# VITA-Group/CV_A-FAN

Measured on AMD Instinct MI355X. Metric: images/sec (whole node) A-FAN K=5 train step, ResNet-18/CIFAR-10, higher is better.
Workload: dtype bf16; 1 GPU; resnet18 CIFAR-10-shape A-FAN K=5 bf16, batch 256/GPU, perturb_idx 6, internal layout nhwc, 1xMI355X per rank (BASELINE configs[1]); global_batch=256, parallelism=dp1, hipgraph=True, in_launch_batchnorm=True

## Files before the change

### cv_a-fan_amd/_lib.py

```python
import ctypes as C
import os

_HERE = os.path.dirname(os.path.abspath(__file__))
LIB_PATH = os.environ.get("AFAN_HIP_LIB") or os.path.join(_HERE, "libafan_hip.so")

AFAN_F32, AFAN_BF16 = 0, 1
AFAN_NCHW, AFAN_NHWC = 0, 1
_ERRORS = {-1: "AFAN_EDTYPE (unknown dtype code)", -2: "AFAN_EALIGN (misaligned pointer)",
           -3: "AFAN_ESHAPE (bad sizes)", -4: "AFAN_ENULL (required pointer is NULL)",
           -5: "AFAN_ELAYOUT (unknown layout code)"}

_p, _i, _l, _f = C.c_void_p, C.c_int, C.c_int64, C.c_float

SIGNATURES = {
    "afan_version": (_i, []),
    "afan_arch": (C.c_char_p, []),
    "afan_pgd_step": (_i, [_p, _p, _i, _p, _p, _l, _f, _f, _i, _p]),
    "afan_tensor_clamp": (_i, [_p, _p, _p, _l, _p]),
    "afan_norms_workspace_floats": (_l, [_l, _l]),
    "afan_pgd_step_norms": (_i, [_p, _p, _i, _p, _p, _l, _l, _f, _f, _i, _p, _p, _p, _p]),
    "afan_perturb_norms": (_i, [_p, _p, _l, _l, _p, _p, _p, _p]),
    "afan_axpy_noise": (_i, [_p, _p, _l, _f, _p, _p]),
    "afan_mix_feature": (_i, [_p, _p, _p, _l, _l, _l, _f, _i, _p]),
    "afan_mix_feature_nhwc": (_i, [_p, _p, _p, _l, _l, _l, _f, _i, _p]),
# ... 113 lines not shown
    "afan_roi_align_bwd_ws": (_i, [_p, _p, _p, _i, _i, _l, _l, _l, _l, _l, _i, _i, _f, _i, _p, _p]),
    "afan_transpose_weights": (_i, [_p, _p, _p, _i, _l, _p]),
    "afan_sgd_step": (_i, [_p, _p, _p, _p, _l, _p, _f, _f, _f, _i, _p]),
    "afan_sgd_step_guarded": (_i, [_p, _p, _p, _p, _l, _p, _f, _f, _f, _i, _p, _p]),
    "afan_guarded_copy": (_i, [_p, _p, _l, _p, _p, _p]),
    "afan_occupy_cus": (_i, [_i, _i, _i, _p]),
    "afan_cast_bf16": (_i, [_p, _p, _l, _p]),
    "afan_pgd_init": (_i, [_p, _i, _p, _p, _p, _l, _p]),
    "afan_normalize_nchw": (_i, [_p, _p, _i, _i, _l, _l, _l, _p, _p, _p]),
    "afan_profile_enable": (_i, [_i]),
    "afan_profile_collect": (_i, [C.c_char_p, C.POINTER(_l), C.POINTER(C.c_double), C.POINTER(C.c_double),
                                  C.POINTER(C.c_double), _i]),
    "afan_profile_event_overhead": (_i, [_i, C.POINTER(_f), _p]),
    "afan_conv_trace": (_i, [_i]),
    "afan_conv_trace_read": (_i, [C.POINTER(_l), C.c_char_p, _i]),
}

_lib = None


class AfanLibraryError(RuntimeError):
    pass


def load():
    global _lib
    if _lib is not None:
        return _lib
    if not os.path.exists(LIB_PATH):
        raise AfanLibraryError(
# ... 18 lines not shown
```

### cv_a-fan_amd/csrc/afan_conv.hip

```cpp
#include "afan_common.h"
#include "afan_conv_c64.h"
#include "afan_conv_stem.h"
#include "afan_conv_params.h"
#include <stdlib.h>

#ifndef AFAN_CONV_DRES_EARLY
#define AFAN_CONV_DRES_EARLY 1
#endif
#ifndef AFAN_CONV_FRAG_BATCH
#define AFAN_CONV_FRAG_BATCH 4
#endif

using namespace afan;
using namespace afan_conv;

namespace afan_nhwc {
int acc_slot_count(int64_t C);
int64_t acc_doubles(int64_t C);
int set_running_updates(int n);
}

namespace {

typedef __bf16 bf16x8 __attribute__((ext_vector_type(8)));
// ... 58 lines not shown

template <int KG, int BR> struct HaloSched {
    static constexpr int s(int t) { return (t < 0 || t >= 7) ? 0 : KG / 7 + (t < KG % 7 ? 1 : 0); }
    static constexpr int g0(int t) { int g = 0; for (int i = 0; i < t; ++i) g += s(i); return g; }
    static constexpr int slot(int tp, bool more) { return tp < 0 ? BR : ((tp + 3 < 9 || more) ? BR : 0) + (more ? s(tp) : 0); }
    static constexpr int wait(int t, bool more) { return slot(t - 1, more) + slot(t - 2, more); }
};

template <int KG, int BR> struct HaloSched5 {
    static constexpr int s(int t) { return (t < 0 || t >= 5) ? 0 : KG / 5 + (t < KG % 5 ? 1 : 0); }
    static constexpr int g0(int t) { int g = 0; for (int i = 0; i < t; ++i) g += s(i); return g; }
    static constexpr int slot(int tp, bool more) { return tp < 0 ? BR : ((tp + 5 < 9 || more) ? BR : 0) + (more ? s(tp) : 0); }
    static constexpr int wait(int t, bool more) { return slot(t - 1, more) + slot(t - 2, more) + slot(t - 3, more); }
};

template <int BM, int BN, int PF, int WM, int WN, int PW = 0, int FBT = AFAN_CONV_FRAG_BATCH, int HL = 0, bool GS = false, bool BF = false>
__device__ __forceinline__ void conv_igemm_body(const ConvP& pp) {
    static_assert(!(BF && GS), "in-launch BatchNorm: one image group");
    AFAN_PHASE(0);
    constexpr int NW = WM * WN;
    constexpr int THREADS = 64 * (NW + PW);
    constexpr int STG = PW ? 64 * PW : THREADS;
    constexpr int RPP = STG / 8;
    const ConvClass& cc = pp.cls[blockIdx.z];
    const uint32_t Wg = (uint32_t)cc.Wg, Hg = (uint32_t)cc.Hg;
    const uint32_t M = (uint32_t)pp.N * Hg * Wg;
    const uint32_t m0 = blockIdx.y * BM;
    if (m0 >= M) {
        if (pp.stats && threadIdx.x < BN && (int)(blockIdx.x * BN + threadIdx.x) < pp.Co) {
            const int64_t G = (int64_t)gridDim.y * gridDim.z, slot = (int64_t)blockIdx.z * gridDim.y + blockIdx.y;
            const int c = blockIdx.x * BN + threadIdx.x;
            pp.stats[((int64_t)0 * pp.Co + c) * G + slot] = 0.f;
            pp.stats[((int64_t)1 * pp.Co + c) * G + slot] = 0.f;
// ... 14 lines not shown

    const int tid = threadIdx.x, lane = tid & 63;
    const int wave = PW ? __builtin_amdgcn_readfirstlane(tid >> 6) : tid >> 6;
    const int wr = wave / WN, wc = wave % WN;
    const bool producer = PW && wave >= NW;
    const int stid = PW ? tid - 64 * NW : tid, swave = PW ? wave - NW : wave;
    const int n0 = blockIdx.x * BN;
    const int T = cc.T, Ci = pp.Ci, Hi = pp.Hi, Wi = pp.Wi;
    int tdh[MAX_TAPS], tdw[MAX_TAPS];
#pragma unroll
    for (int t = 0; t < MAX_TAPS; ++t) {
        tdh[t] = HL ? 0 : cc.dh[t];
        tdw[t] = HL ? 0 : cc.dw[t];
    }
    const int tap0_w = cc.wofs[0], tap0_a = cc.aofs[0], tap0_h = cc.dh[0], tap0_d = cc.dw[0];

    const __amdgpu_buffer_rsrc_t xr = __builtin_amdgcn_make_buffer_rsrc(
        const_cast<uint16_t*>(pp.x), 0, (int)((int64_t)pp.N * Hi * Wi * Ci * 2 + pp.a_extra), 0x00020000);
    const int w_row_stride = pp.multi ? pp.w_rs[blockIdx.z] : pp.w_row_stride;
    const __amdgpu_buffer_rsrc_t wrs = __builtin_amdgcn_make_buffer_rsrc(
        const_cast<uint16_t*>(pp.w + pp.w_off[blockIdx.z]), 0, (int)((int64_t)pp.Co * w_row_stride * 2), 0x00020000);
    constexpr uint32_t OOB = 0x80000000u;

    const int piece = GLDS ? ((stid & 7) ^ ((stid >> 4) & 7)) : (stid & 7);
    const int row0 = stid >> 3;
    uint32_t a_off[A_ROWS];
    uint32_t a_valid[A_ROWS];
#pragma unroll
    for (int i = 0; i < A_ROWS; ++i) {
        const uint32_t m = m0 + row0 + RPP * i;
        a_off[i] = 0;
        a_valid[i] = 0;
        if (!HL && m < M && (!PW || producer)) {
            const uint32_t t1 = m / Wg, wg = m - t1 * Wg;
            const uint32_t n = t1 / Hg, hg = t1 - n * Hg;
            const int hi0 = (int)hg * pp.in_s, wi0 = (int)wg * pp.in_s;
            a_off[i] = (((n * Hi + hi0) * Wi + wi0) * Ci + piece * 8) * 2u;
            uint32_t v = 0;
#pragma unroll
            for (int t = 0; t < MAX_TAPS; ++t)
                if ((t < T) & ((uint32_t)(hi0 + tdh[t]) < (uint32_t)Hi) & ((uint32_t)(wi0 + tdw[t]) < (uint32_t)Wi)) v |= 1u << t;
            a_valid[i] = v;
        }
    }
    __shared__ float coef_s[3][BN];
    float cv0 = 0.f, cv1 = 0.f, cv2 = 0.f;
    if (tid < BN) {
        const int c = n0 + tid < pp.Co ? n0 + tid : 0;
        const uint32_t half_ = (uint32_t)(pp.N / 2) * Hg * Wg;
        const int64_t o_ = c + (m0 >= half_ ? pp.coef_gofs : 0);
        const int64_t o0_ = o_ + ((pp.coef_mask & 8) ? pp.shift_off[blockIdx.z] : 0);
        cv0 = pp.coef[0][o0_];
        cv1 = pp.coef[1][o_];
        cv2 = pp.coef[2][o_];
    }
    auto late_prologue = [&]() {
        for (int r = tid; r < BM; r += THREADS) {
            const uint32_t m = m0 + r;
            int off = -1;
            if (m < M) {
                const uint32_t t1 = m / Wg, wg = m - t1 * Wg;
                const uint32_t n = t1 / Hg, hg = t1 - n * Hg;
                off = (int)(((n * pp.Ho + hg * pp.out_s + cc.out_h0) * pp.Wo + wg * pp.out_s + cc.out_w0) * pp.Co);
            }
            out_off[r] = off;
        }
        if (tid < BN) {
            const int mask_ = pp.coef_mask;
            coef_s[0][tid] = (mask_ & 1) ? cv0 : 0.f;
            coef_s[1][tid] = (mask_ & 2) ? cv1 : 0.f;
            coef_s[2][tid] = (mask_ & 4) ? cv2 : 0.f;
        }
    };
    const uint32_t b_off = ((uint32_t)(n0 + row0) * w_row_stride + piece * 8) * 2u;
    const int b_rows_ok = pp.Co - n0 - row0;
    const uint32_t b_row32 = (uint32_t)RPP * w_row_stride * 2u;

    f32x16 acc[NI][MI];
#pragma unroll
    for (int j = 0; j < NI; ++j)
#pragma unroll
        for (int i = 0; i < MI; ++i)
#pragma unroll
            for (int r = 0; r < 16; ++r) acc[j][i][r] = 0.f;

    const int chunks = (Ci + BK - 1) / BK;
    const int KS = T * chunks;
    const bool last_ok = (chunks - 1) * BK + piece * 8 < Ci;
    u32x4 ra0[A_ROWS], rb0[B_ROWS], ra1[A_ROWS], rb1[B_ROWS];

    auto gload = [&](int ks, u32x4 (&ra)[A_ROWS], u32x4 (&rb)[B_ROWS]) {
        const int q = ks / T, t = ks - q * T;
        const uint32_t a_tap = (uint32_t)(((cc.dh[t] * Wi + cc.dw[t]) * Ci + q * BK + cc.aofs[t]) * 2);
        const uint32_t b_tap = (uint32_t)((cc.wofs[t] + q * BK) * 2);
        const bool pk = q + 1 < chunks || last_ok;
#pragma unroll
        for (int i = 0; i < A_ROWS; ++i) {
            const uint32_t off = (((a_valid[i] >> t) & 1u) && pk) ? a_off[i] + a_tap : OOB;
            ra[i] = __builtin_bit_cast(u32x4, __builtin_amdgcn_raw_buffer_load_b128(xr, (int)off, 0, 0));
        }
#pragma unroll
        for (int i = 0; i < B_ROWS; ++i)
            rb[i] = __builtin_bit_cast(u32x4, __builtin_amdgcn_raw_buffer_load_b128(wrs, (pk && RPP * i < b_rows_ok) ? (int)(b_off + i * b_row32) : (int)OOB, (int)b_tap, 0));
    };
    auto lstore = [&](int buf, const u32x4 (&ra)[A_ROWS], const u32x4 (&rb)[B_ROWS]) {
        uint16_t* A = lds + buf * STAGE;
        uint16_t* B = A + BM * LDK;
#pragma unroll
        for (int i = 0; i < A_ROWS; ++i)
            *reinterpret_cast<u32x4*>(A + (row0 + RPP * i) * LDK + piece * 8) = ra[i];
#pragma unroll
        for (int i = 0; i < B_ROWS; ++i)
            *reinterpret_cast<u32x4*>(B + (row0 + RPP * i) * LDK + piece * 8) = rb[i];
    };
    auto compute = [&](int buf) {
        const uint16_t* A = lds + buf * STAGE;
        const uint16_t* B = A + BM * LDR;
        const int frow = lane & 31, fk = (lane >> 5) * 8;
        const int sw = (frow >> 1) & 7;
        constexpr int FB = FBT;
#pragma unroll
        for (int k0 = 0; k0 < BK / 16; k0 += FB) {
            bf16x8 fx[FB][MI], fw[FB][NI];
#pragma unroll
            for (int b = 0; b < FB; ++b) {
                const int kk = k0 + b;
                const int koff = GLDS ? (((kk * 2 + (lane >> 5)) ^ sw) * 8) : (kk * 16 + fk);
#pragma unroll
                for (int i = 0; i < MI; ++i)
                    fx[b][i] = *reinterpret_cast<const bf16x8*>(A + (wr * TM + i * 32 + frow) * LDR + koff);
#pragma unroll
                for (int j = 0; j < NI; ++j)
                    fw[b][j] = *reinterpret_cast<const bf16x8*>(B + (wc * TN + j * 32 + frow) * LDR + koff);
            }
            if (FB > 1) __builtin_amdgcn_sched_barrier(0);
// ... 3 lines not shown
                for (int j = 0; j < NI; ++j)
#pragma unroll
                    for (int i = 0; i < MI; ++i)
                        acc[j][i] = __builtin_amdgcn_mfma_f32_32x32x16_bf16(fw[b][j], fx[b][i], acc[j][i], 0, 0, 0);
            if (FB > 1) __builtin_amdgcn_sched_barrier(0);
        }
    };


    const uint32_t A_BIAS = (uint32_t)(((pp.max_pad * Wi + pp.max_pad) * Ci) * 2);
    const __amdgpu_buffer_rsrc_t xdma = __builtin_amdgcn_make_buffer_rsrc(
        reinterpret_cast<char*>(const_cast<uint16_t*>(pp.x)) - A_BIAS, 0, (int)((int64_t)pp.N * Hi * Wi * Ci * 2 + A_BIAS + pp.a_extra), 0x00020000);
    uint32_t b_voff[B_ROWS];
#pragma unroll
    for (int i = 0; i < B_ROWS; ++i) b_voff[i] = RPP * i < b_rows_ok ? b_off + i * b_row32 : OOB;
    int dma_t = 0, dma_q = 0;
    int tap_a = T > 0 ? (tap0_h * Wi + tap0_d) * Ci + tap0_a : 0;
    int tap_b = T > 0 ? tap0_w : 0;
    auto gdma = [&](int , int buf) {
        const int t = dma_t;
        const int a_tap = (tap_a + dma_q * BK) * 2 + (int)A_BIAS, b_tap = (tap_b + dma_q * BK) * 2;
        const bool pk = dma_q + 1 < chunks || last_ok;
        uint16_t* A = lds + buf * STAGE + swave * 512;
        uint16_t* B = A + BM * LDR;
        typedef __attribute__((address_space(3))) void* lptr;
#pragma unroll
        for (int i = 0; i < A_ROWS; ++i) {
            const uint32_t voff = (((a_valid[i] >> t) & 1u) && pk) ? a_off[i] : OOB;
            __builtin_amdgcn_raw_ptr_buffer_load_lds(xdma, (lptr)(A + i * (RPP * 64)), 16, (int)voff, a_tap, 0, 0);
        }
#pragma unroll
        for (int i = 0; i < B_ROWS; ++i)
            __builtin_amdgcn_raw_ptr_buffer_load_lds(wrs, (lptr)(B + i * (RPP * 64)), 16, pk ? (int)b_voff[i] : (int)OOB, b_tap, 0, 0);
        if (++dma_t == T) {
            dma_t = 0;
            ++dma_q;
        }
        tap_a = (cc.dh[dma_t] * Wi + cc.dw[dma_t]) * Ci + cc.aofs[dma_t];
        tap_b = cc.wofs[dma_t];
    };

    if constexpr (HL > 0) {
        static_assert(PW == 4 && GLDS && (NS == 4 || NS == 6), "halo form: FOUR producer waves (hdma's group index is k * 4 + swave), four weight stages (or six: the one-tap-ahead form)");
        static_assert(HL <= 448, "halo form: the next chunk's halo must be issued within 7 K-steps (at most 2 groups x 4 waves x 8 pixels each)");
        constexpr int HPM = HL;
        uint16_t* const Hbase = lds + NS * STAGE;
        uint16_t* const pad_zone = Hbase + 2 * HPM * BK;
        typedef __attribute__((address_space(3))) void* lptr;
        const uint32_t W2 = Wg + 2, H2 = Hg + 2;
        auto p0 = [&](uint32_t m) -> int {
            const uint32_t t1 = m / Wg, x = m - t1 * Wg;
            const uint32_t n = t1 / Hg, y = t1 - n * Hg;
            return (int)((n * H2 + y) * W2 + x);
        };
// ... 215 lines not shown
            }
        }
        }
        __syncthreads();
#ifdef AFAN_CONV_STAMP
        if (stamp_on)
            for (int i = 0; i < 96; ++i)
                for (int k = 0; k < 3; ++k) afan_stamps[0][i][k] = (i < chunks * 9 && i < 72) ? st_lds[i][k] : 0ull;
        __syncthreads();
#endif
    } else if constexpr (PW > 0) {
        static_assert(GLDS, "producer waves: LDS-DMA only");
        AFAN_PHASE(1);
        constexpr int LPT = A_ROWS + B_ROWS;
        if constexpr (NS == 2) {
            if (producer) {
                gdma(0, 0);
                __builtin_amdgcn_s_waitcnt(vmcnt_imm(0));
                __builtin_amdgcn_s_barrier();
                for (int ks = 0; ks < KS; ++ks) {
                    if (ks + 1 < KS) gdma(ks + 1, (ks & 1) ^ 1);
                    __builtin_amdgcn_s_waitcnt(vmcnt_imm(0));
                    __builtin_amdgcn_s_barrier();
                }
            } else {
                late_prologue();
                __builtin_amdgcn_s_barrier();
                for (int ks = 0; ks < KS; ++ks) {
                    compute(ks & 1);
                    __builtin_amdgcn_s_waitcnt(0xc07f);
                    __builtin_amdgcn_s_barrier();
                }
            }
            __syncthreads();
        } else
        {
        if (producer) {
#pragma unroll
            for (int s = 0; s < NS - 1; ++s)
                if (s < KS) gdma(s, s);
            int buf = 0;
            for (int ks = 0; ks < KS; ++ks) {
                const int rem = KS - 1 - ks;
                if (rem >= NS - 2) __builtin_amdgcn_s_waitcnt(vmcnt_imm(LPT * (NS - 2)));
                else if (NS == 4 && rem == 1) __builtin_amdgcn_s_waitcnt(vmcnt_imm(LPT));
                else __builtin_amdgcn_s_waitcnt(vmcnt_imm(0));
                __builtin_amdgcn_s_barrier();
                if (ks + NS - 1 < KS) gdma(ks + NS - 1, buf == 0 ? NS - 1 : buf - 1);
                buf = buf + 1 == NS ? 0 : buf + 1;
            }
        } else {
#ifdef AFAN_CONV_PRIO
            __builtin_amdgcn_s_setprio(AFAN_CONV_PRIO);
#endif
            late_prologue();
            int buf = 0;
            for (int ks = 0; ks < KS; ++ks) {
                __builtin_amdgcn_s_barrier();
                compute(buf);
                buf = buf + 1 == NS ? 0 : buf + 1;
            }
        }
        __syncthreads();
        }
    } else if constexpr (GLDS && NS > 2) {
        AFAN_PHASE(1);
        constexpr int LPT = A_ROWS + B_ROWS;
#pragma unroll
        for (int s = 0; s < NS - 1; ++s)
            if (s < KS) gdma(s, s);
        late_prologue();
        int buf = 0;
        for (int ks = 0; ks < KS; ++ks) {
            const int rem = KS - 1 - ks;
            if (rem >= NS - 2) __builtin_amdgcn_s_waitcnt(vmcnt_imm(LPT * (NS - 2)));
            else if (NS == 4 && rem == 1) __builtin_amdgcn_s_waitcnt(vmcnt_imm(LPT));
            else __builtin_amdgcn_s_waitcnt(vmcnt_imm(0));
            __builtin_amdgcn_s_barrier();
            if (ks + NS - 1 < KS) gdma(ks + NS - 1, buf == 0 ? NS - 1 : buf - 1);
            compute(buf);
            buf = buf + 1 == NS ? 0 : buf + 1;
        }
        __syncthreads();
    } else if constexpr (GLDS) {
        AFAN_PHASE(1);
        gdma(0, 0);
        late_prologue();
        __syncthreads();
        for (int ks = 0; ks < KS; ++ks) {
            const int buf = ks & 1;
            if (ks + 1 < KS) gdma(ks + 1, buf ^ 1);
            compute(buf);
            __syncthreads();
        }
    } else if constexpr (PF == 1) {
        late_prologue();
        gload(0, ra0, rb0);
        lstore(0, ra0, rb0);
        __syncthreads();
        for (int ks = 0; ks < KS; ++ks) {
            const int buf = ks & 1;
            if (ks + 1 < KS) gload(ks + 1, ra0, rb0);
            compute(buf);
            if (ks + 1 < KS) lstore(buf ^ 1, ra0, rb0);
            __syncthreads();
        }
    } else {
        late_prologue();
        gload(0, ra0, rb0);
        lstore(0, ra0, rb0);
        if (KS > 1) gload(1, ra1, rb1);
        __syncthreads();
        for (int ks = 0; ks < KS; ks += 2) {
            if (ks + 2 < KS) gload(ks + 2, ra0, rb0);
            compute(0);
            if (ks + 1 < KS) lstore(1, ra1, rb1);
            __syncthreads();
            if (ks + 1 < KS) {
                if (ks + 3 < KS) gload(ks + 3, ra1, rb1);
                compute(1);
                if (ks + 2 < KS) lstore(0, ra0, rb0);
                __syncthreads();
            }
        }
    }

    AFAN_PHASE(2);
    constexpr int LDC = BN + 8;
    uint16_t* C = lds;
    uint16_t* const Z = lds + BM * LDC;
    constexpr bool DRES_EARLY = AFAN_CONV_DRES_EARLY != 0;
    constexpr bool BSC_OK = BF && HL > 0;
    bool have_bsc = false;
    __shared__ float zmean_s[BF ? BN : 1];
    unsigned bar_target = 0;
    if constexpr (BF) {
        if (tid == 0) bar_target = grid_episode(pp.bar);
        have_bsc = BSC_OK && pp.bnf == 2 && pp.bsc.x != nullptr;
        if (have_bsc && tid < BN) zmean_s[tid] = n0 + tid < pp.Co ? pp.bsc.stats[n0 + tid] : 0.f;
        if (have_bsc) {
            constexpr int PIECES_Z = BN / 8, NZ = BM * BN * 2 / 1024;
// ... 437 lines not shown
#pragma unroll
                            for (int j = 0; j < 8; ++j)
                                o[j] = f2bf(fmaf(bf2f(v[j]), pp.bsc.stats[2 * pp.Co + n0 + pc * 8 + j], fmaf(bf2f(zv[j]) - zmean_s[pc * 8 + j], k2[j], k3[j])));
                            *reinterpret_cast<u16x8*>(pp.bsc.y3 + go) = o;
                        }
                    }
                }
            }
            AFAN_PHASE(7);
        }
    }
    }
    AFAN_PHASE(8);
}

template <int BM, int BN, int PF, int WM, int WN, int PW = 0, int FBT = AFAN_CONV_FRAG_BATCH, int HL = 0, bool GS = false, bool BF = false>
__global__ __launch_bounds__(64 * (WM * WN + PW)) void conv_igemm_fwd_kernel(const ConvP pp) {
    conv_igemm_body<BM, BN, PF, WM, WN, PW, FBT, HL, GS, BF>(pp);
}
template <int BM, int BN, int PF, int WM, int WN, int PW = 0, int FBT = AFAN_CONV_FRAG_BATCH, int HL = 0, bool GS = false, bool BF = false>
__global__ __launch_bounds__(64 * (WM * WN + PW)) void conv_igemm_dgrad_kernel(const ConvP pp) {
    conv_igemm_body<BM, BN, PF, WM, WN, PW, FBT, HL, GS, BF>(pp);
}

static int64_t max_rows(const ConvP& p) {
    int64_t m = 0;
    for (int c = 0; c < p.n_classes; ++c) {
        const int64_t v = (int64_t)p.N * p.cls[c].Hg * p.cls[c].Wg;
        if (v > m) m = v;
    }
    return m;
}

// ... 14 lines not shown
    }
    if (ws && p.shift) {
        p.coef[0] = p.shift;
        p.coef_mask |= 1 | 8;
    }
    if (p.aff) {
        p.coef[1] = p.aff + (p.aff_bwd ? 0 : 2 * (int64_t)p.Co);
        p.coef_mask |= 2;
        if (!p.aff_bwd) {
            p.coef[2] = p.aff + 3 * (int64_t)p.Co;
            p.coef_mask |= 4;
        }
    }
}

template <int BM, int BN, int PF, int WM, int WN, int PW, int FBT, int HL, bool GS, bool BF = false>
int launch_gs(const ConvP& p_in, hipStream_t st, bool dgrad) {
    ConvP p = p_in;
    fill_coef(p);
    constexpr int THREADS = 64 * (WM * WN + PW);
    const int64_t M = max_rows(p);
    dim3 grid((unsigned)((p.Co + BN - 1) / BN), (unsigned)((M + BM - 1) / BM), (unsigned)p.n_classes);
    constexpr size_t stage_bytes = HL ? (size_t)(PF - 1) * BN * BK * 2 + (size_t)2 * HL * BK * 2 + 1024
                                      : (size_t)(PF <= 3 ? 2 : PF - 1) * (BM + BN) * (PF >= 3 ? BK : LDK) * 2;
    constexpr size_t epi_bytes = (size_t)BM * (BN + 8) * 2;
    constexpr size_t lds = stage_bytes > epi_bytes ? stage_bytes : epi_bytes;
    static bool attr_done = false;
    if (!attr_done && lds > 64 * 1024) {
        hipError_t e = hipFuncSetAttribute((const void*)conv_igemm_fwd_kernel<BM, BN, PF, WM, WN, PW, FBT, HL, GS, BF>,
                                           hipFuncAttributeMaxDynamicSharedMemorySize, (int)lds);
        if (e == hipSuccess)
            e = hipFuncSetAttribute((const void*)conv_igemm_dgrad_kernel<BM, BN, PF, WM, WN, PW, FBT, HL, GS, BF>,
                                    hipFuncAttributeMaxDynamicSharedMemorySize, (int)lds);
        if (e != hipSuccess) return (int)e;
        attr_done = true;
    }
    if constexpr (BF) {
        static int max_resident = -1, n_cus = 0;
        if (max_resident < 0) {
            int dev = 0, cus = 0, of = 0, od = 0;
            if (hipGetDevice(&dev) != hipSuccess || hipDeviceGetAttribute(&cus, hipDeviceAttributeMultiprocessorCount, dev) != hipSuccess ||
                hipOccupancyMaxActiveBlocksPerMultiprocessor(&of, (const void*)conv_igemm_fwd_kernel<BM, BN, PF, WM, WN, PW, FBT, HL, GS, BF>, THREADS, lds) != hipSuccess ||
                hipOccupancyMaxActiveBlocksPerMultiprocessor(&od, (const void*)conv_igemm_dgrad_kernel<BM, BN, PF, WM, WN, PW, FBT, HL, GS, BF>, THREADS, lds) != hipSuccess)
                return AFAN_ESHAPE;
            n_cus = cus;
            max_resident = cus * (of < od ? of : od);
        }
        const int64_t cap = afan_conv::g_bnf_one_per_cu ? (max_resident < n_cus ? max_resident : n_cus) : max_resident;
        if (p.acc_ns > 8) return AFAN_ESHAPE;
        if (HL == 0 && p.bsc.x) return AFAN_ESHAPE;
        const int64_t meet = (int64_t)grid.x * grid.y * (p.multi ? 1 : grid.z);
        if (meet > cap || meet < 8 || !p.bar || !p.acc || p.groups != 1 || (p.multi && (p.bnf != 1 || p.bnf_sc.acc || p.bnf_res)))
            return AFAN_ESHAPE;
        for (int z = 1; z < p.n_classes; ++z)
            if (p.cls[z].Hg != p.cls[0].Hg || p.cls[z].Wg != p.cls[0].Wg) return AFAN_ESHAPE;
        if (p.n_classes != 1 && !p.multi && (p.bnf != 2 || p.bsc.x)) return AFAN_ESHAPE;
    }
    if (dgrad) conv_igemm_dgrad_kernel<BM, BN, PF, WM, WN, PW, FBT, HL, GS, BF><<<grid, THREADS, lds, st>>>(p);
    else conv_igemm_fwd_kernel<BM, BN, PF, WM, WN, PW, FBT, HL, GS, BF><<<grid, THREADS, lds, st>>>(p);
    AFAN_LAUNCH_CHECK();
    AFAN_TRACE_LAUNCH("igemm_%s<%d,%d,%d,%d,%d,%d,%d,%d,gs%d,bf%d>", dgrad ? "dgrad" : "fwd", BM, BN, PF, WM, WN, PW, FBT, HL, (int)GS, (int)BF);
    return AFAN_OK;
}

template <int BM, int BN, int PF, int WM, int WN, int PW = 0, int FBT = AFAN_CONV_FRAG_BATCH, int HL = 0>
int launch(const ConvP& p, hipStream_t st, bool dgrad) {
    bool gs = false;
    if (p.groups == 2)
        for (int z = 0; z < p.n_classes; ++z) gs = gs || ((int64_t)(p.N / 2) * p.cls[z].Hg * p.cls[z].Wg) % BM != 0;
    constexpr bool GS_BUILT = BM <= 128 && WM * WN + PW <= 12;
    if (gs) {
        if constexpr (GS_BUILT) return launch_gs<BM, BN, PF, WM, WN, PW, FBT, HL, true>(p, st, dgrad);
        else return AFAN_ESHAPE;
    }
    return launch_gs<BM, BN, PF, WM, WN, PW, FBT, HL, false>(p, st, dgrad);
// ... 34 lines not shown
    thread_local Seen seen[NSEEN];
    thread_local int n_seen = 0, next_seen = 0;
    for (int i = 0; i < n_seen; ++i)
        if (seen[i].n == p.N && seen[i].h == H && seen[i].w == W && seen[i].bm == bm && seen[i].cap == cap) return seen[i].ok;
    auto p0 = [&](int64_t m) { const int64_t t1 = m / W, x = m % W, n = t1 / H, y = t1 % H; return (n * (H + 2) + y) * (W + 2) + x; };
    const int64_t tiles = (M + bm - 1) / bm, walk = tiles < 4096 ? tiles : 4096;
    bool ok = tiles <= 4096;
    for (int64_t i = 0; ok && i < walk; ++i) {
        const int64_t m0 = i * bm, m1 = (m0 + bm < M ? m0 + bm : M) - 1;
        if (p0(m1) + 2 * (W + 2) + 2 - p0(m0) + 1 > cap) ok = false;
    }
    seen[next_seen] = Seen{p.N, H, W, bm, cap, ok};
    next_seen = (next_seen + 1) % NSEEN;
    if (n_seen < NSEEN) ++n_seen;
    return ok;
}

#ifndef AFAN_CONV_BNF_TU
int dispatch(const ConvP& p, hipStream_t st, bool dgrad) {
    static const int mode = env_int("AFAN_CONV_MODE", 3);
    static const int force_bm = env_int("AFAN_CONV_BM", 0);
    static const int nw = env_int("AFAN_CONV_NW", 8);
    const int bm = force_bm ? force_bm : choose_bm(max_rows(p), p.Co, p.n_classes, p.multi != 0);
    const bool n128 = p.Co % 128 == 0;
    static const int deep = env_int("AFAN_CONV_DEEP", 1);
    if (mode == 3 && nw >= 8 && n128 && deep >= 1) {
        const int64_t wgs = (int64_t)(p.Co / 128) * ((max_rows(p) + bm - 1) / bm) * p.n_classes;
        static const int deep_max = env_int("AFAN_CONV_DEEPMAX", 256);
        static const int spec = env_int("AFAN_CONV_SPEC", 1);
        static const int halo = env_int("AFAN_CONV_HALO", 1);
// ... 188 lines not shown
    if (bnf) return nc == 4 ? dispatch_bnf(p, st, true) : AFAN_ESHAPE;
    if (!dy_sc && small_eligible(p)) return (p.aff || !small_groups_ok(p)) ? AFAN_ESHAPE : small_launch(p, st);
    if (co % 8 != 0 || ci % 8 != 0 || co < 40 || ci < 40) return AFAN_ESHAPE;
    return dispatch(p, st, true);
}

}

extern "C" {

#ifdef AFAN_CONV_STAMP
int afan_conv_stamps(unsigned long long* host_out) {
    return (int)hipMemcpyFromSymbol(host_out, HIP_SYMBOL(afan_stamps), sizeof(unsigned long long) * 2 * 96 * 3);
}
#endif

int afan_conv_supported(int64_t ci, int64_t co, int k, int stride) {
    if (ci == 3) return afan_stem::eligible(1, 1, 32, ci, co, k, stride) ? 1 : 0;
    return (channels_ok(ci, co) && channels_ok(co, ci) && (k == 1 || k == 3) && (stride == 1 || stride == 2)) ? 1 : 0;
}

int64_t afan_conv_fwd_tiles(int64_t n, int64_t hi, int64_t wi, int64_t ci, int64_t co, int k, int stride) {
    if (check_dims(n, hi, wi, ci, co, k, stride)) return 0;
    const int pad = k / 2;
    const int64_t M = n * ((hi + 2 * pad - k) / stride + 1) * ((wi + 2 * pad - k) / stride + 1);
    const int bm = choose_bm(M, (int)co, 1);
    return (M + bm - 1) / bm;
}

int afan_conv_fwd_nhwc_bf16(const void* x, const void* w, void* y, int64_t n, int64_t hi, int64_t wi, int64_t ci,
// ... 406 lines not shown
```

### cv_a-fan_amd/csrc/afan_conv_bnf.hip

```cpp
#define AFAN_CONV_BNF_TU 1
#include "afan_conv.hip"

}

namespace afan_conv {

int g_bnf_one_per_cu = 0;

int dispatch_bnf(const ConvP& p, hipStream_t st, bool dgrad) {
    static const int halo = env_int("AFAN_CONV_HALO", 1);
    if (!halo || p.Co % 128 != 0 || p.stats || !p.acc || p.groups != 1) return AFAN_ESHAPE;
    const int bm = choose_bm(max_rows(p), p.Co, p.n_classes, p.multi != 0);
    const int64_t wgs = (int64_t)(p.Co / 128) * ((max_rows(p) + bm - 1) / bm) * p.n_classes;
    constexpr int deep_max = 384;
    static const int ahead = env_int("AFAN_CONV_AHEAD", 1);
    static const int t64 = env_int("AFAN_CONV_T64", 1);
    if (t64 && p.n_classes == 1 && p.Ci >= 128) {
        const int64_t w64 = (int64_t)(p.Co / 64) * ((max_rows(p) + 63) / 64);
        if (w64 <= 256 && w64 >= 16) {
            static const int ahead64 = env_int("AFAN_CONV_AHEAD64", 1);
            if (halo_ok(p, 64))
                return ahead64 ? launch_gs<64, 64, 7, 2, 2, 4, AFAN_CONV_FRAG_BATCH, HALO_PIXELS, false, true>(p, st, dgrad)
                               : launch_gs<64, 64, 5, 2, 2, 4, AFAN_CONV_FRAG_BATCH, HALO_PIXELS, false, true>(p, st, dgrad);
            return launch_gs<64, 64, 5, 2, 2, 4, AFAN_CONV_FRAG_BATCH, 0, false, true>(p, st, dgrad);
// ... 10 lines not shown
    if (bm == 128 && wgs <= deep_max && p.Ci >= 256) {
        const int64_t wgs_n64 = (int64_t)(p.Co / 64) * ((max_rows(p) + 255) / 256) * p.n_classes;
        static const int w41 = env_int("AFAN_CONV_W41", 1);
        if (wgs_n64 <= deep_max && wgs_n64 >= wgs && halo_ok(p, 256, HALO_PIXELS_256N))
            return !w41 ? launch_gs<256, 64, 5, 4, 2, 4, 2, HALO_PIXELS_256N, false, true>(p, st, dgrad)
                        : (ahead ? launch_gs<256, 64, 7, 4, 1, 4, 2, HALO_PIXELS_256N, false, true>(p, st, dgrad)
                                 : launch_gs<256, 64, 5, 4, 1, 4, 2, HALO_PIXELS_256N, false, true>(p, st, dgrad));
    }
    if (wgs <= deep_max && halo_ok(p, bm))
        return bm == 64 ? launch_gs<64, 128, 5, 2, 2, 4, AFAN_CONV_FRAG_BATCH, HALO_PIXELS, false, true>(p, st, dgrad)
                        : launch_gs<128, 128, 5, 2, 2, 4, AFAN_CONV_FRAG_BATCH, HALO_PIXELS, false, true>(p, st, dgrad);
    static const int tap3 = env_int("AFAN_BNF_TAP3", 1);
    if (!tap3 && p.cls[0].T == 9) return AFAN_ESHAPE;
    if (wgs <= deep_max) {
        const int e = bm == 64 ? launch_gs<64, 128, 5, 2, 2, 4, AFAN_CONV_FRAG_BATCH, 0, false, true>(p, st, dgrad)
                               : launch_gs<128, 128, 5, 2, 2, 4, AFAN_CONV_FRAG_BATCH, 0, false, true>(p, st, dgrad);
        if (e != AFAN_ESHAPE) return e;
    }
    return bm == 64 ? launch_gs<64, 128, 3, 2, 4, 0, AFAN_CONV_FRAG_BATCH, 0, false, true>(p, st, dgrad)
                    : launch_gs<128, 128, 3, 2, 4, 0, AFAN_CONV_FRAG_BATCH, 0, false, true>(p, st, dgrad);
}

}

#ifdef AFAN_CONV_STAMP
extern "C" int afan_conv_bnf_stamps(unsigned long long* host_out) {
    return (int)hipMemcpyFromSymbol(host_out, HIP_SYMBOL(afan_stamps), sizeof(unsigned long long) * 2 * 96 * 3);
}
#endif
```

### cv_a-fan_amd/csrc/afan_conv_params.h

```cpp
#pragma once
#include "afan_common.h"

namespace afan_conv {

constexpr int MAX_TAPS = 9;

struct ConvClass {
    int Hg, Wg;
    int out_h0, out_w0;
    int T;
    int dh[MAX_TAPS], dw[MAX_TAPS], wofs[MAX_TAPS];
    int aofs[MAX_TAPS];
};

struct ConvP {
    const uint16_t* x;
    const uint16_t* w;
    uint16_t* y;
    int N, Hi, Wi, Ci;
    int Ho, Wo, Co;
    int in_s;
    int out_s;
    int w_row_stride;
    int n_classes;
// ... 52 lines not shown
    float* bnf_dw;
    float* bnf_db;
    int bnf_accum;
    struct BSc {
        const uint16_t* x;
        const float* stats;
        double* acc;
        uint16_t* y3;
        float* dw;
        float* db;
    } bsc;
};

int dispatch_bnf(const ConvP& p, hipStream_t st, bool dgrad);
extern int g_bnf_one_per_cu;


bool small_eligible(const ConvP& p);
int small_launch(const ConvP& p, hipStream_t st);

}
```

### cv_a-fan_amd/ops.py

```python
import ctypes as C
import os
import threading

import torch

from . import _lib
from ._lib import AFAN_BF16, AFAN_F32, AFAN_NCHW, AFAN_NHWC, AfanLibraryError, check

_DT = {torch.float32: AFAN_F32, torch.bfloat16: AFAN_BF16}
_ws_cache = {}
_tls = threading.local()
CALLS = {"conv_fwd": 0, "conv_dgrad": 0, "conv_wgrad": 0, "conv_general": 0, "vendor_conv": 0, "conv_bn_fused": 0}


def _need(t, name, dtype=None):
    if not isinstance(t, torch.Tensor):
        raise TypeError(f"{name}: expected a torch.Tensor")
    if t.device.type != "cuda":
        raise AfanLibraryError(f"{name}: tensor is on '{t.device}'. The A-FAN kernels are MI355X-only; "
                               "there is no CPU path (the CPU restatement under oracle/ is test infrastructure).")
    if not _dense(t):
        raise ValueError(f"{name}: tensor must be dense (contiguous NCHW or channels_last)")
    if dtype is not None and t.dtype != dtype:
        raise TypeError(f"{name}: expected {dtype}, got {t.dtype}")
# ... 1786 lines not shown


class conv_trace:

    def __init__(self):
        self.records = []

    def __enter__(self):
        check(_lib.load().afan_conv_trace(1), "afan_conv_trace")
        return self

    def __exit__(self, *exc):
        check(_lib.load().afan_conv_trace(0), "afan_conv_trace")
        self.records = _conv_trace_read()
        return False
```

### include/afan_hip.h

```cpp
#ifndef AFAN_HIP_H
#define AFAN_HIP_H

#include <stdint.h>

#ifdef __cplusplus
extern "C" {
#endif

typedef void* afan_stream_t;

enum { AFAN_F32 = 0, AFAN_BF16 = 1 };

enum { AFAN_NCHW = 0, AFAN_NHWC = 1 };

enum {
    AFAN_OK = 0,
    AFAN_EDTYPE = -1,
    AFAN_EALIGN = -2,
    AFAN_ESHAPE = -3,
    AFAN_ENULL = -4,
    AFAN_ELAYOUT = -5
};

int afan_version(void);
// ... 301 lines not shown
int afan_occupy_cus(int workgroups, int lds_bytes, int microseconds, afan_stream_t stream);

int afan_cast_bf16(const float* src, uint16_t* dst, int64_t n, afan_stream_t stream);
int afan_pgd_init(const void* x, int dtype, float* x32, float* x_adv, uint16_t* shadow, int64_t n, afan_stream_t stream);
int afan_normalize_nchw(const float* x, void* y, int out_dtype, int out_layout, int64_t n, int64_t c, int64_t hw,
                        const float* mean, const float* std, afan_stream_t stream);

int afan_profile_enable(int on);
int afan_profile_collect(char* names_out, int64_t* launches, double* total_ms, double* total_bytes,
                         double* total_flops, int max_kernels);
int afan_profile_event_overhead(int n, float* us_out, afan_stream_t stream);

int afan_conv_trace(int on);
int afan_conv_trace_read(int64_t* problems, char* names, int max_records);

#ifdef __cplusplus
}
#endif
#endif
```

Measured before the change: 34550 images/sec.

## Fuse 1x1 projection shortcut into the 3x3 conv tile as an extra tap

Adds a PAIR variant of the in-launch-BatchNorm implicit-GEMM forward kernel. For a two-class multi launch (3x3 conv plus 1x1 downsample projection), one block now computes both outputs over the same A tile: the projection is treated as a tenth tap that accumulates into a second register accumulator. This replaces the grid z dimension of two classes with a single class, which shares input loads and halves the block count. The cost is doubled accumulator registers, a smaller fragment batch, a forced waves-per-EU hint, and a separate epilogue that writes the projection output and its BN statistics. The variant is declined when the unpaired grid already fits twice in the resident cap, and a debug hook reporting the last grid is also added.

```diff
diff --git a/cv_a-fan_amd/_lib.py b/cv_a-fan_amd/_lib.py
--- a/cv_a-fan_amd/_lib.py
+++ b/cv_a-fan_amd/_lib.py
@@ -151,6 +151,7 @@
     "afan_profile_event_overhead": (_i, [_i, C.POINTER(_f), _p]),
     "afan_conv_trace": (_i, [_i]),
     "afan_conv_trace_read": (_i, [C.POINTER(_l), C.c_char_p, _i]),
+    "afan_conv_last_grid": (_i, [C.POINTER(_i)]),
 }
 
 _lib = None
diff --git a/cv_a-fan_amd/csrc/afan_conv.hip b/cv_a-fan_amd/csrc/afan_conv.hip
--- a/cv_a-fan_amd/csrc/afan_conv.hip
+++ b/cv_a-fan_amd/csrc/afan_conv.hip
@@ -96,9 +96,10 @@
     static constexpr int wait(int t, bool more) { return slot(t - 1, more) + slot(t - 2, more) + slot(t - 3, more); }
 };
 
-template <int BM, int BN, int PF, int WM, int WN, int PW = 0, int FBT = AFAN_CONV_FRAG_BATCH, int HL = 0, bool GS = false, bool BF = false>
+template <int BM, int BN, int PF, int WM, int WN, int PW = 0, int FBT = AFAN_CONV_FRAG_BATCH, int HL = 0, bool GS = false, bool BF = false, bool PAIR = false>
 __device__ __forceinline__ void conv_igemm_body(const ConvP& pp) {
     static_assert(!(BF && GS), "in-launch BatchNorm: one image group");
+    static_assert(!PAIR || (BF && HL == 0 && PF >= 3 && (PW == 0 ? PF == 3 : PF > 3)), "paired projection: the two per-tap in-launch-BatchNorm forms");
     AFAN_PHASE(0);
     constexpr int NW = WM * WN;
     constexpr int THREADS = 64 * (NW + PW);
@@ -143,6 +144,9 @@
         tdw[t] = HL ? 0 : cc.dw[t];
     }
     const int tap0_w = cc.wofs[0], tap0_a = cc.aofs[0], tap0_h = cc.dh[0], tap0_d = cc.dw[0];
+    const ConvClass& c1 = pp.cls[PAIR ? 1 : 0];
+    const int pr_h = c1.dh[0], pr_d = c1.dw[0], pr_w = c1.wofs[0];
+    const int TT = PAIR ? T + 1 : T;
 
     const __amdgpu_buffer_rsrc_t xr = __builtin_amdgcn_make_buffer_rsrc(
         const_cast<uint16_t*>(pp.x), 0, (int)((int64_t)pp.N * Hi * Wi * Ci * 2 + pp.a_extra), 0x00020000);
@@ -169,11 +173,13 @@
 #pragma unroll
             for (int t = 0; t < MAX_TAPS; ++t)
                 if ((t < T) & ((uint32_t)(hi0 + tdh[t]) < (uint32_t)Hi) & ((uint32_t)(wi0 + tdw[t]) < (uint32_t)Wi)) v |= 1u << t;
+            if (PAIR && ((uint32_t)(hi0 + pr_h) < (uint32_t)Hi) & ((uint32_t)(wi0 + pr_d) < (uint32_t)Wi)) v |= 1u << T;
             a_valid[i] = v;
         }
     }
     __shared__ float coef_s[3][BN];
-    float cv0 = 0.f, cv1 = 0.f, cv2 = 0.f;
+    __shared__ float coef_p[PAIR ? BN : 1];
+    float cv0 = 0.f, cv1 = 0.f, cv2 = 0.f, cvp = 0.f;
     if (tid < BN) {
         const int c = n0 + tid < pp.Co ? n0 + tid : 0;
         const uint32_t half_ = (uint32_t)(pp.N / 2) * Hg * Wg;
@@ -182,6 +188,7 @@
         cv0 = pp.coef[0][o0_];
         cv1 = pp.coef[1][o_];
         cv2 = pp.coef[2][o_];
+        if constexpr (PAIR) cvp = pp.coef[0][o_ + ((pp.coef_mask & 8) ? pp.shift_off[1] : 0)];
     }
     auto late_prologue = [&]() {
         for (int r = tid; r < BM; r += THREADS) {
@@ -199,6 +206,7 @@
             coef_s[0][tid] = (mask_ & 1) ? cv0 : 0.f;
             coef_s[1][tid] = (mask_ & 2) ? cv1 : 0.f;
             coef_s[2][tid] = (mask_ & 4) ? cv2 : 0.f;
+            if constexpr (PAIR) coef_p[tid] = (mask_ & 1) ? cvp : 0.f;
         }
     };
     const uint32_t b_off = ((uint32_t)(n0 + row0) * w_row_stride + piece * 8) * 2u;
@@ -206,15 +214,19 @@
     const uint32_t b_row32 = (uint32_t)RPP * w_row_stride * 2u;
 
     f32x16 acc[NI][MI];
+    f32x16 acc2[NI][MI];
 #pragma unroll
     for (int j = 0; j < NI; ++j)
 #pragma unroll
         for (int i = 0; i < MI; ++i)
 #pragma unroll
-            for (int r = 0; r < 16; ++r) acc[j][i][r] = 0.f;
+            for (int r = 0; r < 16; ++r) {
+                acc[j][i][r] = 0.f;
+                if constexpr (PAIR) acc2[j][i][r] = 0.f;
+            }
 
     const int chunks = (Ci + BK - 1) / BK;
-    const int KS = T * chunks;
+    const int KS = TT * chunks;
     const bool last_ok = (chunks - 1) * BK + piece * 8 < Ci;
     u32x4 ra0[A_ROWS], rb0[B_ROWS], ra1[A_ROWS], rb1[B_ROWS];
 
@@ -242,12 +254,12 @@
         for (int i = 0; i < B_ROWS; ++i)
             *reinterpret_cast<u32x4*>(B + (row0 + RPP * i) * LDK + piece * 8) = rb[i];
     };
-    auto compute = [&](int buf) {
+    auto compute = [&](int buf, f32x16 (&acc)[NI][MI]) {
         const uint16_t* A = lds + buf * STAGE;
         const uint16_t* B = A + BM * LDR;
         const int frow = lane & 31, fk = (lane >> 5) * 8;
         const int sw = (frow >> 1) & 7;
-        constexpr int FB = FBT;
+        constexpr int FB = (PAIR && PW == 0 && MI * NI >= 2 && FBT > 2) ? 2 : FBT;
 #pragma unroll
         for (int k0 = 0; k0 < BK / 16; k0 += FB) {
             bf16x8 fx[FB][MI], fw[FB][NI];
@@ -281,6 +293,15 @@
     uint32_t b_voff[B_ROWS];
 #pragma unroll
     for (int i = 0; i < B_ROWS; ++i) b_voff[i] = RPP * i < b_rows_ok ? b_off + i * b_row32 : OOB;
+    const int w_rs1 = pp.w_rs[PAIR ? 1 : 0];
+    const __amdgpu_buffer_rsrc_t wrs1 = __builtin_amdgcn_make_buffer_rsrc(
+        const_cast<uint16_t*>(pp.w + pp.w_off[PAIR ? 1 : 0]), 0, (int)((int64_t)pp.Co * w_rs1 * 2), 0x00020000);
+    uint32_t b_voff1[PAIR ? B_ROWS : 1];
+    if constexpr (PAIR) {
+#pragma unroll
+        for (int i = 0; i < B_ROWS; ++i)
+            b_voff1[i] = RPP * i < b_rows_ok ? ((uint32_t)(n0 + row0 + RPP * i) * w_rs1 + piece * 8) * 2u : OOB;
+    }
     int dma_t = 0, dma_q = 0;
     int tap_a = T > 0 ? (tap0_h * Wi + tap0_d) * Ci + tap0_a : 0;
     int tap_b = T > 0 ? tap0_w : 0;
@@ -296,15 +317,23 @@
             const uint32_t voff = (((a_valid[i] >> t) & 1u) && pk) ? a_off[i] : OOB;
             __builtin_amdgcn_raw_ptr_buffer_load_lds(xdma, (lptr)(A + i * (RPP * 64)), 16, (int)voff, a_tap, 0, 0);
         }
-#pragma unroll
-        for (int i = 0; i < B_ROWS; ++i)
-            __builtin_amdgcn_raw_ptr_buffer_load_lds(wrs, (lptr)(B + i * (RPP * 64)), 16, pk ? (int)b_voff[i] : (int)OOB, b_tap, 0, 0);
-        if (++dma_t == T) {
+        if (PAIR && t == T) {
+#pragma unroll
+            for (int i = 0; i < B_ROWS; ++i)
+                __builtin_amdgcn_raw_ptr_buffer_load_lds(wrs1, (lptr)(B + i * (RPP * 64)), 16, pk ? (int)b_voff1[PAIR ? i : 0] : (int)OOB, b_tap, 0, 0);
+        } else {
+#pragma unroll
+            for (int i = 0; i < B_ROWS; ++i)
+                __builtin_amdgcn_raw_ptr_buffer_load_lds(wrs, (lptr)(B + i * (RPP * 64)), 16, pk ? (int)b_voff[i] : (int)OOB, b_tap, 0, 0);
+        }
+        if (++dma_t == TT) {
             dma_t = 0;
             ++dma_q;
         }
-        tap_a = (cc.dh[dma_t] * Wi + cc.dw[dma_t]) * Ci + cc.aofs[dma_t];
-        tap_b = cc.wofs[dma_t];
+        const bool np = PAIR && dma_t == T;
+        const int ti = np ? 0 : dma_t;
+        tap_a = np ? (pr_h * Wi + pr_d) * Ci : (cc.dh[ti] * Wi + cc.dw[ti]) * Ci + cc.aofs[ti];
+        tap_b = np ? pr_w : cc.wofs[ti];
     };
 
     if constexpr (HL > 0) {
@@ -550,6 +579,7 @@
         AFAN_PHASE(1);
         constexpr int LPT = A_ROWS + B_ROWS;
         if constexpr (NS == 2) {
+            static_assert(!PAIR, "paired projection: not in this form");
             if (producer) {
                 gdma(0, 0);
                 __builtin_amdgcn_s_waitcnt(vmcnt_imm(0));
@@ -563,7 +593,7 @@
                 late_prologue();
                 __builtin_amdgcn_s_barrier();
                 for (int ks = 0; ks < KS; ++ks) {
-                    compute(ks & 1);
+                    compute(ks & 1, acc);
                     __builtin_amdgcn_s_waitcnt(0xc07f);
                     __builtin_amdgcn_s_barrier();
                 }
@@ -591,15 +621,28 @@
 #endif
             late_prologue();
             int buf = 0;
+            if constexpr (PAIR) {
+                for (int q = 0; q < chunks; ++q) {
+                    for (int t = 0; t < T; ++t) {
+                        __builtin_amdgcn_s_barrier();
+                        compute(buf, acc);
+                        buf = buf + 1 == NS ? 0 : buf + 1;
+                    }
+                    __builtin_amdgcn_s_barrier();
+                    compute(buf, acc2);
+                    buf = buf + 1 == NS ? 0 : buf + 1;
+                }
+            } else
             for (int ks = 0; ks < KS; ++ks) {
                 __builtin_amdgcn_s_barrier();
-                compute(buf);
+                compute(buf, acc);
                 buf = buf + 1 == NS ? 0 : buf + 1;
             }
         }
         __syncthreads();
         }
     } else if constexpr (GLDS && NS > 2) {
+        static_assert(!PAIR, "paired projection: not in this form");
         AFAN_PHASE(1);
         constexpr int LPT = A_ROWS + B_ROWS;
 #pragma unroll
@@ -614,7 +657,7 @@
             else __builtin_amdgcn_s_waitcnt(vmcnt_imm(0));
             __builtin_amdgcn_s_barrier();
             if (ks + NS - 1 < KS) gdma(ks + NS - 1, buf == 0 ? NS - 1 : buf - 1);
-            compute(buf);
+            compute(buf, acc);
             buf = buf + 1 == NS ? 0 : buf + 1;
         }
         __syncthreads();
@@ -623,10 +666,24 @@
         gdma(0, 0);
         late_prologue();
         __syncthreads();
+        if constexpr (PAIR) {
+            int ks = 0;
+            for (int q = 0; q < chunks; ++q) {
+                for (int t = 0; t < T; ++t, ++ks) {
+                    gdma(ks + 1, (ks & 1) ^ 1);
+                    compute(ks & 1, acc);
+                    __syncthreads();
+                }
+                if (ks + 1 < KS) gdma(ks + 1, (ks & 1) ^ 1);
+                compute(ks & 1, acc2);
+                __syncthreads();
+                ++ks;
+            }
+        } else
         for (int ks = 0; ks < KS; ++ks) {
             const int buf = ks & 1;
             if (ks + 1 < KS) gdma(ks + 1, buf ^ 1);
-            compute(buf);
+            compute(buf, acc);
             __syncthreads();
         }
     } else if constexpr (PF == 1) {
@@ -637,7 +694,7 @@
         for (int ks = 0; ks < KS; ++ks) {
             const int buf = ks & 1;
             if (ks + 1 < KS) gload(ks + 1, ra0, rb0);
-            compute(buf);
+            compute(buf, acc);
             if (ks + 1 < KS) lstore(buf ^ 1, ra0, rb0);
             __syncthreads();
         }
@@ -649,18 +706,95 @@
         __syncthreads();
         for (int ks = 0; ks < KS; ks += 2) {
             if (ks + 2 < KS) gload(ks + 2, ra0, rb0);
-            compute(0);
+            compute(0, acc);
             if (ks + 1 < KS) lstore(1, ra1, rb1);
             __syncthreads();
             if (ks + 1 < KS) {
                 if (ks + 3 < KS) gload(ks + 3, ra1, rb1);
-                compute(1);
+                compute(1, acc);
                 if (ks + 2 < KS) lstore(0, ra0, rb0);
                 __syncthreads();
             }
         }
     }
 
+    if constexpr (PAIR) {
+        constexpr int LDC_P = BN + 8, PIECES_P = BN / 8, ROWS_P = THREADS / PIECES_P, EPI_P = BM / ROWS_P;
+        static_assert((THREADS & (THREADS - 1)) == 0 && BM % ROWS_P == 0, "paired projection: every thread stores");
+        static_assert((size_t)BM * LDC_P * 2 + (size_t)(THREADS / 64) * 2 * BN * 4 <= (size_t)NS * STAGE * 2, "paired projection: tile + partial sums in the stage buffers");
+        uint16_t* Cp = lds;
+        float (*redp)[2][BN] = reinterpret_cast<float (*)[2][BN]>(lds + BM * LDC_P);
+        if (!producer)
+#pragma unroll
+        for (int j = 0; j < NI; ++j)
+#pragma unroll
+            for (int i = 0; i < MI; ++i) {
+                const int pix = wr * TM + i * 32 + (lane & 31);
+#pragma unroll
+                for (int g = 0; g < 4; ++g) {
+                    const int ch = wc * TN + j * 32 + 8 * g + 4 * (lane >> 5);
+                    u16x4 v;
+#pragma unroll
+                    for (int e = 0; e < 4; ++e) v[e] = f2bf(acc2[j][i][4 * g + e]);
+                    *reinterpret_cast<u16x4*>(Cp + pix * LDC_P + ch) = v;
+                }
+            }
+        __syncthreads();
+        const int pc = tid % PIECES_P, pr = tid / PIECES_P;
+        const bool ch_ok = n0 + pc * 8 < pp.Co;
+        uint16_t* const y1 = pp.y + pp.y_off[1];
+        float s1[8], s2[8], sh[8];
+#pragma unroll
+        for (int j = 0; j < 8; ++j) {
+            s1[j] = s2[j] = 0.f;
+            sh[j] = coef_p[pc * 8 + j];
+        }
+#pragma unroll
+        for (int q = 0; q < EPI_P; ++q) {
+            const int r = pr + q * ROWS_P;
+            const int off = out_off[r];
+            if (off >= 0 && ch_ok) {
+                const u16x8 v = *reinterpret_cast<const u16x8*>(Cp + r * LDC_P + pc * 8);
+                *reinterpret_cast<u16x8*>(y1 + (int64_t)off + n0 + pc * 8) = v;
+#pragma unroll
+                for (int j = 0; j < 8; ++j) {
+                    const float f = bf2f(v[j]) - sh[j];
+                    s1[j] += f;
+                    s2[j] += f * f;
+                }
+            }
+        }
+#pragma unroll
+        for (int o = PIECES_P; o < 64; o <<= 1)
+#pragma unroll
+            for (int j = 0; j < 8; ++j) {
+                s1[j] += __shfl_xor(s1[j], o, 64);
+                s2[j] += __shfl_xor(s2[j], o, 64);
+            }
+        if (lane < PIECES_P) {
+#pragma unroll
+            for (int j = 0; j < 8; ++j) {
+                redp[wave][0][lane * 8 + j] = s1[j];
+                redp[wave][1][lane * 8 + j] = s2[j];
+            }
+        }
+        __syncthreads();
+        if (tid < BN && n0 + tid < pp.Co) {
+            float a = 0.f, b = 0.f;
+#pragma unroll
+            for (int w = 0; w < THREADS / 64; ++w) {
+                a += redp[w][0][tid];
+                b += redp[w][1][tid];
+            }
+            double* const blk = pp.acc + pp.acc_off[1];
+            double* dst = blk + (int64_t)((blockIdx.y + 1) & (pp.acc_ns - 1)) * 2 * pp.Co;
+            unsafeAtomicAdd(dst + n0 + tid, (double)a);
+            unsafeAtomicAdd(dst + pp.Co + n0 + tid, (double)b);
+            if (m0 == 0)
+                reinterpret_cast<float*>(blk + (int64_t)2 * pp.acc_ns * pp.Co)[n0 + tid] = pp.shift ? pp.shift[pp.shift_off[1] + n0 + tid] : 0.f;
+        }
+        __syncthreads();
+    }
     AFAN_PHASE(2);
     constexpr int LDC = BN + 8;
     uint16_t* C = lds;
@@ -1128,9 +1262,10 @@
     AFAN_PHASE(8);
 }
 
-template <int BM, int BN, int PF, int WM, int WN, int PW = 0, int FBT = AFAN_CONV_FRAG_BATCH, int HL = 0, bool GS = false, bool BF = false>
-__global__ __launch_bounds__(64 * (WM * WN + PW)) void conv_igemm_fwd_kernel(const ConvP pp) {
-    conv_igemm_body<BM, BN, PF, WM, WN, PW, FBT, HL, GS, BF>(pp);
+template <int BM, int BN, int PF, int WM, int WN, int PW = 0, int FBT = AFAN_CONV_FRAG_BATCH, int HL = 0, bool GS = false, bool BF = false, bool PAIR = false>
+__global__ __launch_bounds__(64 * (WM * WN + PW)) __attribute__((amdgpu_waves_per_eu((PAIR && PW == 0) ? 4 : 1)))
+void conv_igemm_fwd_kernel(const ConvP pp) {
+    conv_igemm_body<BM, BN, PF, WM, WN, PW, FBT, HL, GS, BF, PAIR>(pp);
 }
 template <int BM, int BN, int PF, int WM, int WN, int PW = 0, int FBT = AFAN_CONV_FRAG_BATCH, int HL = 0, bool GS = false, bool BF = false>
 __global__ __launch_bounds__(64 * (WM * WN + PW)) void conv_igemm_dgrad_kernel(const ConvP pp) {
@@ -1175,22 +1310,24 @@
     }
 }
 
-template <int BM, int BN, int PF, int WM, int WN, int PW, int FBT, int HL, bool GS, bool BF = false>
+constexpr int PAIR_DECLINED = -1000;
+template <int BM, int BN, int PF, int WM, int WN, int PW, int FBT, int HL, bool GS, bool BF = false, bool PAIR = false>
 int launch_gs(const ConvP& p_in, hipStream_t st, bool dgrad) {
     ConvP p = p_in;
     fill_coef(p);
     constexpr int THREADS = 64 * (WM * WN + PW);
     const int64_t M = max_rows(p);
-    dim3 grid((unsigned)((p.Co + BN - 1) / BN), (unsigned)((M + BM - 1) / BM), (unsigned)p.n_classes);
+    if (PAIR && dgrad) return AFAN_ESHAPE;
+    dim3 grid((unsigned)((p.Co + BN - 1) / BN), (unsigned)((M + BM - 1) / BM), PAIR ? 1u : (unsigned)p.n_classes);
     constexpr size_t stage_bytes = HL ? (size_t)(PF - 1) * BN * BK * 2 + (size_t)2 * HL * BK * 2 + 1024
                                       : (size_t)(PF <= 3 ? 2 : PF - 1) * (BM + BN) * (PF >= 3 ? BK : LDK) * 2;
     constexpr size_t epi_bytes = (size_t)BM * (BN + 8) * 2;
     constexpr size_t lds = stage_bytes > epi_bytes ? stage_bytes : epi_bytes;
     static bool attr_done = false;
     if (!attr_done && lds > 64 * 1024) {
-        hipError_t e = hipFuncSetAttribute((const void*)conv_igemm_fwd_kernel<BM, BN, PF, WM, WN, PW, FBT, HL, GS, BF>,
+        hipError_t e = hipFuncSetAttribute((const void*)conv_igemm_fwd_kernel<BM, BN, PF, WM, WN, PW, FBT, HL, GS, BF, PAIR>,
                                            hipFuncAttributeMaxDynamicSharedMemorySize, (int)lds);
-        if (e == hipSuccess)
+        if (e == hipSuccess && !PAIR)
             e = hipFuncSetAttribute((const void*)conv_igemm_dgrad_kernel<BM, BN, PF, WM, WN, PW, FBT, HL, GS, BF>,
                                     hipFuncAttributeMaxDynamicSharedMemorySize, (int)lds);
         if (e != hipSuccess) return (int)e;
@@ -1201,16 +1338,17 @@
         if (max_resident < 0) {
             int dev = 0, cus = 0, of = 0, od = 0;
             if (hipGetDevice(&dev) != hipSuccess || hipDeviceGetAttribute(&cus, hipDeviceAttributeMultiprocessorCount, dev) != hipSuccess ||
-                hipOccupancyMaxActiveBlocksPerMultiprocessor(&of, (const void*)conv_igemm_fwd_kernel<BM, BN, PF, WM, WN, PW, FBT, HL, GS, BF>, THREADS, lds) != hipSuccess ||
+                hipOccupancyMaxActiveBlocksPerMultiprocessor(&of, (const void*)conv_igemm_fwd_kernel<BM, BN, PF, WM, WN, PW, FBT, HL, GS, BF, PAIR>, THREADS, lds) != hipSuccess ||
                 hipOccupancyMaxActiveBlocksPerMultiprocessor(&od, (const void*)conv_igemm_dgrad_kernel<BM, BN, PF, WM, WN, PW, FBT, HL, GS, BF>, THREADS, lds) != hipSuccess)
                 return AFAN_ESHAPE;
             n_cus = cus;
-            max_resident = cus * (of < od ? of : od);
+            max_resident = cus * ((of < od || PAIR) ? of : od);
         }
         const int64_t cap = afan_conv::g_bnf_one_per_cu ? (max_resident < n_cus ? max_resident : n_cus) : max_resident;
         if (p.acc_ns > 8) return AFAN_ESHAPE;
         if (HL == 0 && p.bsc.x) return AFAN_ESHAPE;
         const int64_t meet = (int64_t)grid.x * grid.y * (p.multi ? 1 : grid.z);
+        if (PAIR && 2 * meet <= cap) return PAIR_DECLINED;
         if (meet > cap || meet < 8 || !p.bar || !p.acc || p.groups != 1 || (p.multi && (p.bnf != 1 || p.bnf_sc.acc || p.bnf_res)))
             return AFAN_ESHAPE;
         for (int z = 1; z < p.n_classes; ++z)
@@ -1218,8 +1356,9 @@
         if (p.n_classes != 1 && !p.multi && (p.bnf != 2 || p.bsc.x)) return AFAN_ESHAPE;
     }
     if (dgrad) conv_igemm_dgrad_kernel<BM, BN, PF, WM, WN, PW, FBT, HL, GS, BF><<<grid, THREADS, lds, st>>>(p);
-    else conv_igemm_fwd_kernel<BM, BN, PF, WM, WN, PW, FBT, HL, GS, BF><<<grid, THREADS, lds, st>>>(p);
+    else conv_igemm_fwd_kernel<BM, BN, PF, WM, WN, PW, FBT, HL, GS, BF, PAIR><<<grid, THREADS, lds, st>>>(p);
     AFAN_LAUNCH_CHECK();
+    afan_conv::g_last_grid[0] = (int)grid.x; afan_conv::g_last_grid[1] = (int)grid.y; afan_conv::g_last_grid[2] = (int)grid.z;
     AFAN_TRACE_LAUNCH("igemm_%s<%d,%d,%d,%d,%d,%d,%d,%d,gs%d,bf%d>", dgrad ? "dgrad" : "fwd", BM, BN, PF, WM, WN, PW, FBT, HL, (int)GS, (int)BF);
     return AFAN_OK;
 }
@@ -1284,6 +1423,12 @@
     next_seen = (next_seen + 1) % NSEEN;
     if (n_seen < NSEEN) ++n_seen;
     return ok;
+}
+
+static bool pair_ok(const ConvP& p, bool dgrad) {
+    static const int on = env_int("AFAN_CONV_PAIR", 1);
+    return on && !dgrad && p.multi && p.n_classes == 2 && p.bnf == 1 && p.cls[0].T == 9 && p.cls[1].T == 1 && !p.a_extra &&
+           p.cls[1].aofs[0] == 0 && p.cls[0].Hg == p.cls[1].Hg && p.cls[0].Wg == p.cls[1].Wg && p.acc && p.groups == 1;
 }
 
 #ifndef AFAN_CONV_BNF_TU
@@ -1502,6 +1647,12 @@
     return (int)hipMemcpyFromSymbol(host_out, HIP_SYMBOL(afan_stamps), sizeof(unsigned long long) * 2 * 96 * 3);
 }
 #endif
+
+int afan_conv_last_grid(int* xyz) {
+    if (!xyz) return AFAN_ENULL;
+    for (int i = 0; i < 3; ++i) xyz[i] = afan_conv::g_last_grid[i];
+    return AFAN_OK;
+}
 
 int afan_conv_supported(int64_t ci, int64_t co, int k, int stride) {
     if (ci == 3) return afan_stem::eligible(1, 1, 32, ci, co, k, stride) ? 1 : 0;
diff --git a/cv_a-fan_amd/csrc/afan_conv_bnf.hip b/cv_a-fan_amd/csrc/afan_conv_bnf.hip
--- a/cv_a-fan_amd/csrc/afan_conv_bnf.hip
+++ b/cv_a-fan_amd/csrc/afan_conv_bnf.hip
@@ -6,6 +6,16 @@
 namespace afan_conv {
 
 int g_bnf_one_per_cu = 0;
+int g_last_grid[3] = {0, 0, 0};
+
+template <int BM, int PF, int WN, int PW>
+static int launch_tap(const ConvP& p, hipStream_t st, bool dgrad) {
+    if (pair_ok(p, dgrad)) {
+        const int e = launch_gs<BM, 128, PF, 2, WN, PW, AFAN_CONV_FRAG_BATCH, 0, false, true, true>(p, st, dgrad);
+        if (e != PAIR_DECLINED) return e;
+    }
+    return launch_gs<BM, 128, PF, 2, WN, PW, AFAN_CONV_FRAG_BATCH, 0, false, true>(p, st, dgrad);
+}
 
 int dispatch_bnf(const ConvP& p, hipStream_t st, bool dgrad) {
     static const int halo = env_int("AFAN_CONV_HALO", 1);
@@ -48,11 +58,11 @@
     if (!tap3 && p.cls[0].T == 9) return AFAN_ESHAPE;
     if (wgs <= deep_max) {
         const int e = bm == 64 ? launch_gs<64, 128, 5, 2, 2, 4, AFAN_CONV_FRAG_BATCH, 0, false, true>(p, st, dgrad)
-                               : launch_gs<128, 128, 5, 2, 2, 4, AFAN_CONV_FRAG_BATCH, 0, false, true>(p, st, dgrad);
+                               : launch_tap<128, 5, 2, 4>(p, st, dgrad);
         if (e != AFAN_ESHAPE) return e;
     }
     return bm == 64 ? launch_gs<64, 128, 3, 2, 4, 0, AFAN_CONV_FRAG_BATCH, 0, false, true>(p, st, dgrad)
-                    : launch_gs<128, 128, 3, 2, 4, 0, AFAN_CONV_FRAG_BATCH, 0, false, true>(p, st, dgrad);
+                    : launch_tap<128, 3, 4, 0>(p, st, dgrad);
 }
 
 }
diff --git a/cv_a-fan_amd/csrc/afan_conv_params.h b/cv_a-fan_amd/csrc/afan_conv_params.h
--- a/cv_a-fan_amd/csrc/afan_conv_params.h
+++ b/cv_a-fan_amd/csrc/afan_conv_params.h
@@ -90,6 +90,7 @@
 
 int dispatch_bnf(const ConvP& p, hipStream_t st, bool dgrad);
 extern int g_bnf_one_per_cu;
+extern int g_last_grid[3];
 
 
 bool small_eligible(const ConvP& p);
diff --git a/cv_a-fan_amd/ops.py b/cv_a-fan_amd/ops.py
--- a/cv_a-fan_amd/ops.py
+++ b/cv_a-fan_amd/ops.py
@@ -1824,3 +1824,9 @@
         check(_lib.load().afan_conv_trace(0), "afan_conv_trace")
         self.records = _conv_trace_read()
         return False
+
+
+def conv_last_grid():
+    g = (C.c_int * 3)()
+    check(_lib.load().afan_conv_last_grid(g), "afan_conv_last_grid")
+    return int(g[0]), int(g[1]), int(g[2])
diff --git a/include/afan_hip.h b/include/afan_hip.h
--- a/include/afan_hip.h
+++ b/include/afan_hip.h
@@ -339,6 +339,8 @@
 int afan_conv_trace(int on);
 int afan_conv_trace_read(int64_t* problems, char* names, int max_records);
 
+int afan_conv_last_grid(int* xyz);
+
 #ifdef __cplusplus
 }
 #endif
```

Result: no change. 34610 images/sec, median of 6 (+0.2%).
